# michaelriedl/2048-ppo-agent

Hardware: AMD Instinct MI355X
Metric: env-steps/sec at N parallel boards (full PPO loop: rollout with policy in the loop + GAE + update) (higher is better)
Workload: dtype u8 boards / bf16 policy; 1 GPU; 65536 parallel boards per GPU, Transformer policy bf16 (3.96 M params), full PPO iteration (BASELINE.json configs[2]; configs[3] when n_gpus=8); boards_per_gpu=65536, global_boards=65536, train_batch=2048, update_epochs=5, max_samples_per_epoch=300000, max_samples_per_epoch_is=global (each rank draws its 1/N share), as the reference's single subset, max_samples_per_epoch_per_rank=300000, rollout_mode=episodes (reference lock-step semantics), rng_mode=partitionable, parallelism=env-shard x1 + 1 grad all-reduce/minibatch

## Files before the change

2048-ppo-agent_amd/csrc/g2048_rowgemm.hip:

```cpp
#include <hip/hip_runtime.h>
#include <stdint.h>
#include <stdlib.h>

#include <type_traits>

#include "../../include/g2048.h"
#include "g2048_mfma.h"

namespace {

using namespace g2048_mfma;

constexpr int RG_N = 256, RG_KC = 128, RG_THREADS = 512, RG_WAVES = 8;
template <int NB> struct RgShape {
    static constexpr int TT = 32 * NB, STAGE = TT * RG_KC * 2, PIECES = TT * (RG_KC / 8) / RG_THREADS, RPW = TT / RG_WAVES, BATCH = RPW / 2;
    static constexpr int LDS = 2 * STAGE + RG_WAVES * 3 * RG_N * 4 + RG_N * 4;
    static_assert(PIECES * RG_THREADS == TT * (RG_KC / 8) && RPW % 2 == 0 && BATCH >= 1, "tile shape");
};

typedef uint32_t u32x4 __attribute__((ext_vector_type(4)));
enum { RG_FWD = 0, RG_BWD = 1 };

struct RowGemmArgs {
    const __bf16 *x;
// ... 312 lines not shown
                red[(w * 3 + 1) * RG_N + 4 * lane + q] = db[q];
                red[(w * 3 + 2) * RG_N + 4 * lane + q] = dsum[q];
            }
            lds_barrier();
            for (int c = tid; c < 3 * RG_N; c += RG_THREADS) {
                float s = 0.f;
#pragma unroll
                for (int ww = 0; ww < RG_WAVES; ++ww) s += red[ww * 3 * RG_N + c];
                float *dst = A.partial + (int64_t)blockIdx.x * 3 * RG_N + c;
                *dst = (tile == (int64_t)blockIdx.x) ? s : *dst + s;
            }
        }
    }
}

inline int rg_done() {
    const hipError_t e = hipGetLastError();
    return e == hipSuccess ? 0 : -(1000 + (int)e);
}

inline int rg_tpw(int64_t T, int *nb) {
    const char *e = getenv("G2048_RG_TWO_TILES");
    const bool two = e && e[0] == '1';
    int64_t t = (T + 255) / 256;
    if (two) t = (T + 511) / 512;
    if (t <= 96 && (two || t <= 48)) {
        *nb = 3;
        return (int)(t < 32 ? 32 : t);
    }
    *nb = 5;
// ... 45 lines not shown
extern "C" int g2048_linear_add_ln_fwd(const void *u, int64_t ldu, const void *w_packed, const float *bias, int K, const float *x,
                                       int64_t x_row_stride, const float *gamma, const float *beta, float *x_new, void *h, float *mean,
                                       float *rstd, int64_t T, float eps, float p_drop, uint64_t seed, const uint64_t *seed_state,
                                       void *stream) {
    if (!rg_gemm_ok(u, ldu, w_packed, T, K) || !x || !gamma || !beta || !x_new || !h || !mean || !rstd || !(p_drop >= 0.f && p_drop < 1.f) ||
        (x_row_stride & 3) || (((uintptr_t)x | (uintptr_t)gamma | (uintptr_t)beta | (uintptr_t)x_new | (uintptr_t)bias) & 15) ||
        ((uintptr_t)h & 7))
        return G2048_EINVAL;
    RowGemmArgs A{};
    A.x = (const __bf16 *)u; A.ldx = ldu; A.w = (const __bf16 *)w_packed; A.bias = bias; A.T = T; A.K = K;
    A.w_tile_stride = (int64_t)(K >> 4) * 512; A.extra_period = 1;
    A.res = x; A.res_rs = x_row_stride; A.gamma = gamma; A.beta = beta; A.mean = mean; A.rstd = rstd; A.out_f32 = x_new;
    A.out_bf16 = (uint16_t *)h; A.eps = eps; A.inv_keep = 1.0f / (1.0f - p_drop); A.thr = (uint32_t)(p_drop * 16777216.0f);
    A.s0 = (uint32_t)seed; A.s1 = (uint32_t)(seed >> 32); A.seed_state = seed_state; A.g_x_period = 1;
    return rg_launch<RG_FWD>(A, (hipStream_t)stream);
}

extern "C" int g2048_linear_add_ln_bwd(const void *dy, int64_t lddy, const void *wt_packed, int64_t wt_tile_stride, int K,
                                       const float *x_norm, int64_t x_row_stride, const float *g_x, int g_x_period, const void *g_h_extra,
                                       int extra_period, const float *mean, const float *rstd, const float *gamma, float *dx, void *da,
                                       float *partial, int64_t T, float p_drop, uint64_t seed, const uint64_t *seed_state, void *stream) {
    if (wt_tile_stride == 0) wt_tile_stride = (int64_t)(K >> 4) * 512;
    if (wt_tile_stride < (int64_t)(K >> 4) * 512 || (wt_tile_stride & 7) || (g_h_extra && extra_period < 1) || ((uintptr_t)g_h_extra & 7))
        return G2048_EINVAL;
    if (!rg_gemm_ok(dy, lddy, wt_packed, T, K) || !x_norm || !mean || !rstd || !gamma || !dx || !partial || g_x_period < 1 ||
        !(p_drop >= 0.f && p_drop < 1.f) || (x_row_stride & 3) ||
        (((uintptr_t)x_norm | (uintptr_t)g_x | (uintptr_t)gamma | (uintptr_t)dx) & 15) || ((uintptr_t)da & 7) || ((uintptr_t)partial & 3))
        return G2048_EINVAL;
    RowGemmArgs A{};
    A.x = (const __bf16 *)dy; A.ldx = lddy; A.w = (const __bf16 *)wt_packed; A.T = T; A.K = K;
// ... 8 lines not shown
```

2048-ppo-agent_amd/src/g2048/native.py:

```python
from __future__ import annotations

import ctypes as C
import os

import numpy as np
import torch

RNG_LEGACY = 0
RNG_PARTITIONABLE = 1
POLICY_DRUL = 0
POLICY_RANDOM = 1
MAX_FUSED_STEPS = 128

_PKG_ROOT = os.path.abspath(os.path.join(os.path.dirname(__file__), "..", ".."))
LIB_PATH = os.environ.get("G2048_LIB", os.path.join(_PKG_ROOT, "lib", "libg2048.so"))

_u32, _i32, _i64, _vp, _dbl = C.c_uint32, C.c_int, C.c_int64, C.c_void_p, C.c_double

SIGNATURES = {
    "g2048_abi_version": [],
    "g2048_split": [_u32, _u32, _vp, _i64, _i32, _vp],
    "g2048_chain_keys": [_vp, _vp, _i64, _i32],
    "g2048_init": [_vp, _vp, _vp, _vp, _i64, _i32, _vp],
    "g2048_step": [_vp, _vp, _vp, _vp, _vp, _vp, _i64, _i32, _vp],
# ... 28 lines not shown
    "g2048_linear_relu_dropout_bf16": [_vp, _i64, _vp, _i64, _vp, _vp, _i64, _i64, _i32, _i32, C.c_float, C.c_uint64, _vp, _vp, _vp],
    "g2048_linear_mask_bwd_workspace_floats": [_i64, _i32],
    "g2048_linear_mask_bwd_bf16": [_vp, _i64, _vp, _i64, _vp, _vp, _i64, _vp, _vp, _i64, _i32, _i32, C.c_float, _vp],
    "g2048_embed_fwd": [_vp, _vp, C.c_int, _vp, _vp, _vp, _i64, C.c_float, C.c_uint64, _vp, _vp],
    "g2048_embed_ln_fwd": [_vp, _vp, C.c_int, _vp, _vp, _vp, _i64, C.c_float, C.c_uint64, _vp, _vp, _vp, C.c_float, _vp, _vp, _vp, _vp],
    "g2048_embed_bwd_workspace_floats": [_i64],
    "g2048_embed_bwd": [_vp, _vp, _vp, _vp, _i64, C.c_float, C.c_uint64, _vp, _vp],
    "g2048_gather_minibatch": [_vp, _i64, _i64] + [_vp] * 13,
    "g2048_colsum_workspace_floats": [_i64, _i32],
    "g2048_colsum": [_vp, _i32, _i64, _i64, _i32, _vp, _vp, _vp],
    "g2048_colsum_partial_rows": [_i64, _i32],
    "g2048_linear_mask_bwd_partial_rows": [_i64, _i32],
    "g2048_reduce_jobs": [_vp, _i32, _vp],
    "g2048_linear_add_ln_fwd": [_vp, _i64, _vp, _vp, _i32, _vp, _i64, _vp, _vp, _vp, _vp, _vp, _vp, _i64, C.c_float, C.c_float,
                                C.c_uint64, _vp, _vp],
    "g2048_linear_add_ln_bwd_partial_rows": [_i64],
    "g2048_linear_add_ln_bwd": [_vp, _i64, _vp, _i64, _i32, _vp, _i64, _vp, _i32, _vp, _i32, _vp, _vp, _vp, _vp, _vp, _vp, _i64,
                                C.c_float, C.c_uint64, _vp, _vp],
    "g2048_mlp_embed_fwd": [_vp, _vp, _vp, _vp, _vp, _i64, _vp],
    "g2048_gemm_jobs": [_vp, _i32, _i64, _vp],
    "g2048_mlp_out_fwd": [_vp, _vp, _vp, _vp, _i64, _vp],
    "g2048_mlp_out_bwd_partial_rows": [_i64],
    "g2048_mlp_out_bwd": [_vp, _vp, _vp, _vp, _vp, _vp, _i64, _vp],
    "g2048_add_ln_bwd_workspace_floats": [_i64],
    "g2048_add_ln_bwd": [_vp, _i64, _vp, _vp, _vp, _vp, _vp, _vp, _vp, _vp, _vp, _i64, C.c_float, C.c_uint64, _vp,
                         _i32, _vp],
    "g2048_relu_dropout_fwd": [_vp, _vp, _i64, _i32, C.c_float, C.c_uint64, _vp, _vp],
    "g2048_relu_dropout_bwd_workspace_floats": [_i64, _i32],
    "g2048_relu_dropout_bwd": [_vp, _vp, _vp, _vp, _vp, _i64, _i32, C.c_float, _vp],
    "g2048_cls_tail_fwd": [_vp, _vp, _i64, _vp, _vp, _vp, _vp, _i64, C.c_float, C.c_float, C.c_uint64, _vp, _vp],
# ... 288 lines not shown


def rowgemm_ok(u2: torch.Tensor, w_packed: torch.Tensor, tile_stride: int = 0) -> bool:
    if u2.dim() != 2 or not u2.is_cuda or u2.dtype != torch.bfloat16 or u2.stride(1) != 1:
        return False
    T, K = u2.shape
    span = 256 * K if not tile_stride else 7 * int(tile_stride) + (K // 16) * 512
    return (T > 0 and K % 256 == 0 and 256 <= K <= 1024 and u2.stride(0) >= K and u2.stride(0) % 8 == 0 and u2.data_ptr() % 16 == 0
            and w_packed is not None and w_packed.is_cuda and w_packed.dtype == torch.bfloat16 and w_packed.is_contiguous()
            and (w_packed.numel() == span if not tile_stride else (w_packed.numel() >= span and tile_stride >= (K // 16) * 512
                                                                  and tile_stride % 8 == 0))
            and w_packed.data_ptr() % 16 == 0 and 160 * u2.stride(0) * 2 < 2 ** 31)


def linear_add_ln_fwd(u2, w_packed, bias, x_ptr: int, x_row_stride: int, gamma, beta, x_new, h, mean, rstd, eps: float,
                      p_drop: float, seed: int, seed_state: int = 0):
    if not rowgemm_ok(u2, w_packed):
        raise NativeError(f"linear_add_ln_fwd: operands {tuple(u2.shape)} (strides {u2.stride()}) x packed {w_packed.numel()} not supported")
    T, K = u2.shape
    bf = torch.bfloat16
    _check(load().g2048_linear_add_ln_fwd(u2.data_ptr(), u2.stride(0), w_packed.data_ptr(), _dev(bias, f32, 256, "bias", optional=True),
                                          K, x_ptr, int(x_row_stride), _dev(gamma, f32, 256, "gamma"), _dev(beta, f32, 256, "beta"),
                                          _dev(x_new, f32, 256 * T, "x_new"), _dev(h, bf, 256 * T, "h"), _dev(mean, f32, T, "mean"),
                                          _dev(rstd, f32, T, "rstd"), T, float(eps), float(p_drop), int(seed), seed_state or None,
                                          _stream()), "g2048_linear_add_ln_fwd")


def linear_add_ln_bwd(dy2, wt_packed, xn_ptr: int, x_row_stride: int, g_x, mean, rstd, gamma, dx, da, p_drop: float, seed: int,
                      seed_state: int = 0, g_x_period: int = 1, tile_stride: int = 0, g_h_extra=None, extra_period: int = 1):
    if not rowgemm_ok(dy2, wt_packed, tile_stride):
        raise NativeError(f"linear_add_ln_bwd: operands {tuple(dy2.shape)} (strides {dy2.stride()}) x packed {wt_packed.numel()} not supported")
# ... 157 lines not shown
    if logits.numel() != 4 * M or values.numel() != M:
        raise NativeError(f"ppo_loss: logits {tuple(logits.shape)} / values {tuple(values.shape)} do not match M={M}")
    new_logp = torch.empty(M, dtype=f32, device=logits.device)
    sums = torch.empty(5, dtype=f32, device=logits.device)
    dlogits, dvalues = torch.empty_like(logits), torch.empty_like(values)
    _check(load().g2048_ppo_loss(
        logits.data_ptr(), int(logits.dtype == torch.bfloat16), values.data_ptr(), int(values.dtype == torch.bfloat16),
        _dev(actions, u8, M, "actions"), _dev(mask_bits, u8, M, "mask_bits", optional=True), _dev(old_logp, f32, M, "old_logp"),
        _dev(adv, f32, M, "adv"), _dev(ret, f32, M, "ret"), M, float(clip_eps), float(c_value), float(c_entropy),
        new_logp.data_ptr(), sums.data_ptr(), dlogits.data_ptr(), dvalues.data_ptr(),
        _dev(grad_scale, f32, 1, "grad_scale", optional=True), _dev(running, torch.float64, 5, "running", optional=True),
        _stream()), "g2048_ppo_loss")
    return new_logp, sums, dlogits, dvalues


def linear_ok(x2: torch.Tensor, weight: torch.Tensor) -> bool:
    return (x2.is_cuda and x2.dtype == torch.bfloat16 and weight.dtype == torch.bfloat16 and x2.dim() == 2
            and weight.dim() == 2 and x2.stride(1) == 1 and weight.stride(1) == 1 and x2.shape[1] == weight.shape[1]
            and x2.shape[1] % 128 == 0 and weight.shape[0] % 128 == 0 and x2.stride(0) % 8 == 0 and weight.stride(0) % 8 == 0
            and x2.data_ptr() % 16 == 0 and weight.data_ptr() % 16 == 0 and x2.shape[0] > 0)


def linear_bf16(x2: torch.Tensor, weight: torch.Tensor, bias_f32=None, out=None) -> torch.Tensor:
    if not linear_ok(x2, weight):
        raise NativeError(f"linear_bf16: unsupported operands {tuple(x2.shape)} {x2.dtype} x {tuple(weight.shape)} {weight.dtype}")
    T, K = x2.shape
    N = weight.shape[0]
    if out is None:
        out = torch.empty((T, N), dtype=torch.bfloat16, device=x2.device)
    _check(load().g2048_linear_bf16(x2.data_ptr(), x2.stride(0), weight.data_ptr(), weight.stride(0),
# ... 317 lines not shown
```

2048-ppo-agent_amd/src/ppo/hip_ops.py:

```python
import weakref

import torch
import torch.nn as nn
import torch.nn.functional as F


class Bf16Shadow:

    _live = weakref.WeakSet()

    def __init__(self, params, transposed=(), packed=(), packed_only=(), packed_t_only=()):
        self.params = list(params)
        self.key, self.flat, self.views = None, None, None
        self.transposed = tuple(transposed)
        self.tviews = {}
        self.packed = tuple(packed)
        self.packed_only, self.packed_t_only = tuple(packed_only), tuple(packed_t_only)
        self.pviews, self.ptviews = {}, {}
        self.maintainer = None
        Bf16Shadow._live.add(self)

    def __getstate__(self):
        return {"params": self.params, "transposed": self.transposed, "packed": self.packed, "packed_only": self.packed_only,
                "packed_t_only": self.packed_t_only}
# ... 200 lines not shown

    def take(self):
        p, self.pending = self.pending, None
        return p


class FFNLink:

    __slots__ = ("p_drop", "db", "masked", "bias_param", "db_sunk", "bits")

    def __init__(self, p_drop: float):
        self.p_drop, self.db, self.masked = float(p_drop), None, False
        self.bits = None
        self.bias_param, self.db_sunk = None, False



_SINK_SLICES = 16


def _dweight_parts(dy2: torch.Tensor, x2: torch.Tensor) -> torch.Tensor:
    T, S = x2.shape[0], _SINK_SLICES
    if T >= 16384:
        from ..g2048 import native as nv

        slices = 16 if dy2.shape[1] * x2.shape[1] > 256 * 256 else 32
        if nv.dweight_ok(dy2, x2, slices):
            return nv.dweight_parts(dy2, x2, slices, block_rows=128)
    if T % S == 0 and T // S >= 64:
        return torch.bmm(dy2.view(S, T // S, -1).transpose(1, 2), x2.view(S, T // S, -1))
# ... 400 lines not shown

    @staticmethod
    def backward(ctx, g):
        if ctx.link is not None:
            ctx.link.g = g.contiguous()
            return None, None
        gx = g.new_zeros(ctx.shape)
        gx[:, :1] = g
        return gx, None


class _LinearAddLayerNorm(torch.autograd.Function):

    @staticmethod
    def forward(ctx, u, weight, bias, wb, bb, x, gamma, beta, eps, p_drop, wbT=None, link=None, cls_link=None, h_link=None,
                w_packed=None):
        from ..g2048 import native as nv

        ctx.set_materialize_grads(False)
        ctx.wbT, ctx.link = wbT, link
        ctx.params = (weight, bias, gamma, beta)
        ctx.cls_link = cls_link
        ctx.h_link = h_link
        if h_link is not None:
            h_link.armed = _rowgemm_on()
        if cls_link is not None:
            cls_link.attached = x.dim() == 3
        x, row_stride = _residual_rows(x)
        T = x.numel() // 256
        gamma, beta = gamma.contiguous(), beta.contiguous()
        h = torch.empty(x.shape, dtype=torch.bfloat16, device=x.device)
        x_new = torch.empty(x.shape, dtype=torch.float32, device=x.device)
        stats = torch.empty((2, T), dtype=torch.float32, device=x.device)
        seed = _seed_pair(x, p_drop)
        u2 = u.reshape(-1, u.shape[-1])
        if (w_packed is not None and _rowgemm_on() and u2.shape[0] == T and T >= 4096 and (bias is None or bias.dtype == torch.float32)
                and nv.rowgemm_ok(u2, w_packed)):
            nv.linear_add_ln_fwd(u2, w_packed, None if bias is None else bias.detach(), x.data_ptr(), row_stride, gamma, beta, x_new, h,
                                 stats[0], stats[1], eps, p_drop, *seed)
        else:
            with torch.autocast("cuda", enabled=False):
                a = _hip_linear(u2, wb, bias.detach()) if bias is not None and u.is_contiguous() else None
                a = F.linear(u, wb, bb) if a is None else a.view(*u.shape[:-1], wb.shape[0])
            nv.add_ln_fwd(x.data_ptr(), row_stride, a, gamma, beta, x_new, h, stats[0], stats[1], T, eps, p_drop, *seed)
        ctx.save_for_backward(u, wb, x_new, gamma, stats)
        ctx.meta = (p_drop, seed)
        return x_new, h

    @staticmethod
    def backward(ctx, g_x, g_h):
        from ..g2048 import native as nv
# ... 37 lines not shown
                if link is not None and link.bits is not None and ctx.wbT is not None and _stationary_ok(da2, ctx.wbT):
                    sink1 = _sink_for(link.bias_param)
                    if sink1 is not None:
                        du, ws1 = nv.linear_mask_bwd(da2, ctx.wbT, link.bits, link.p_drop, final=False)
                        sink1.add(link.bias_param, ws1, ws1.shape[1], ws1.shape[1], ws1.shape[0])
                        link.db, link.db_sunk = None, True
                    else:
                        du, link.db = nv.linear_mask_bwd(da2, ctx.wbT, link.bits, link.p_drop)
                    link.masked, link.bits = True, None
                    du = du.view(u.shape)
                else:
                    du = _hip_linear(da2, ctx.wbT) if ctx.wbT is not None else None
                    du = (da2 @ wb if du is None else du).view(u.shape)
            if sink is not None:
                _sink_weight(sink, weight, da2, u2)
                return du, None, None, None, None, dx, None, None, None, None, None, None, None, None, None
            dw = _dweight(da2, u2)
        return du, dw, dparams[2], None, None, dx, dparams[0], dparams[1], None, None, None, None, None, None, None


class _LinearAddCast(torch.autograd.Function):

    @staticmethod
    def forward(ctx, u, weight, bias, wb, bb, x, p_drop):
        from ..g2048 import native as nv

        with torch.autocast("cuda", enabled=False):
            a = F.linear(u, wb, bb)
        ctx.params = (weight, bias)
        xr, row_stride = _residual_rows(x)
        T = xr.numel() // 256
        h = torch.empty(xr.shape, dtype=torch.bfloat16, device=x.device)
        seed = _seed_pair(xr, p_drop)
# ... 17 lines not shown
        ws = nv.add_ln_bwd(0, 256, None, g_h.contiguous(), None, None, None, dx, da, dparams, T, p_drop, *seed)
        with torch.autocast("cuda", enabled=False):
            da2, u2 = da.view(T, 256), u.reshape(T, -1)
            du = (da2 @ wb).view(u.shape) if ctx.needs_input_grad[0] else None
            if sink is not None:
                sink.add(bias, ws[:, 512:], 768, 256, ws.shape[0])
                _sink_weight(sink, weight, da2, u2)
                return du, None, None, None, None, dx, None
            dw = _dweight(da2, u2)
        return du, dw, dparams[2], None, None, dx, None


class _LinearReluDropout(torch.autograd.Function):

    @staticmethod
    def forward(ctx, h, weight, bias, wb, bb, p_drop, link=None, h_link=None, wt_packed=None):
        from ..g2048 import native as nv

        ctx.h_link, ctx.wt_packed = h_link, wt_packed
        h2 = h.reshape(-1, h.shape[-1])
        with torch.autocast("cuda", enabled=False):
            if _stationary_ok(h2, wb) and bias.dtype == torch.float32:
                y = nv.linear_relu_dropout(h2, wb, bias.detach(), p_drop, *_seed_pair(h2, p_drop), want_mask=link is not None)
                if link is not None:
                    y, link.bits = y
                y = y.view(*h.shape[:-1], wb.shape[0])
            else:
                z = _hip_linear(h2, wb, bias)
                z = F.linear(h, wb, bb) if z is None else z.view(*h.shape[:-1], wb.shape[0])
                y = torch.empty_like(z)
                nv.relu_dropout_fwd(z, y, p_drop, *_seed_pair(z, p_drop))
        ctx.save_for_backward(h, wb, y)
        ctx.p_drop, ctx.link = p_drop, link
        ctx.params = (weight, bias)
        if link is not None:
            link.bias_param = bias
        return y
# ... 14 lines not shown
            dz = torch.empty_like(y)
            db = None if sink is not None else torch.empty(y.shape[-1], dtype=torch.float32, device=y.device)
            ws = nv.relu_dropout_bwd(dy.contiguous(), y, dz, db, ctx.p_drop)
            if sink is not None:
                sink.add(bias, ws, ws.shape[1], ws.shape[1], ws.shape[0])
                db_done = True
        with torch.autocast("cuda", enabled=False):
            dz2, h2 = dz.view(-1, dz.shape[-1]), h.reshape(-1, h.shape[-1])
            dh = None
            if ctx.needs_input_grad[0] and not (ctx.h_link is not None and ctx.h_link.offer(dz2, ctx.wt_packed)):
                dh = (dz2 @ wb).view(h.shape)
            if sink is not None:
                _sink_weight(sink, weight, dz2, h2)
                if not db_done:
                    sink.add(bias, db.contiguous(), db.numel(), db.numel(), 1)
                return dh, None, None, None, None, None, None, None, None
            dw = _dweight(dz2, h2)
        return dh, dw, (None if db_done else db), None, None, None, None, None, None


def _fused_norm_ok(x: torch.Tensor, a) -> bool:
    return (x.is_cuda and x.dtype == torch.float32 and x.shape[-1] == 256 and torch.is_grad_enabled()
            and torch.is_autocast_enabled() and torch.get_autocast_dtype("cuda") == torch.bfloat16
            and (a is None or a.dtype == torch.bfloat16))


def _add_norm(x: torch.Tensor, a, norm: nn.LayerNorm, p: float, training: bool, h_link=None, pre=None):
    if _fused_norm_ok(x, a):
        if a is None and _residual_rows(x)[0] is not x:
            return x, _AddLayerNorm.apply(x, a, norm.weight, norm.bias, norm.eps, 0.0)[1]
        return _AddLayerNorm.apply(x, a, norm.weight, norm.bias, norm.eps, p if training else 0.0, h_link, pre)
    if a is not None:
        x = x + F.dropout(a, p, training)
# ... 199 lines not shown
```

2048-ppo-agent_amd/src/ppo/transformer_encoder.py:

```python
import math
import os

import torch
import torch.nn as nn
import torch.nn.functional as F

from ..env_definitions import BOARD_DIM
from .hip_ops import (Bf16Shadow, ClsLink, FFNLink, HLink, LNPre, _AddLayerNorm, _ClsRows, _AttnCls, _AttnPacked, _EmbedBoards, _ExpandRows, _InProjCls,
                      _LinearAddCast, _LinearAddLayerNorm, _LinearReluDropout, _LinearSplitK, _add_norm, _fused_attention_ok, _fused_norm_ok,
                      _linear, _train_bf16, graph_seed_state)



def get_emb(sin_inp: torch.Tensor) -> torch.Tensor:
    return torch.stack((sin_inp.sin(), sin_inp.cos()), dim=-1).flatten(-2, -1)


class PositionalEncoding2D(nn.Module):

    def __init__(self, x_size, y_size, channels, dropout=0.1, dtype_override=None):
        super().__init__()
        self.org_channels = channels
        self.dtype_override = dtype_override
        self.channels = int(math.ceil(channels / 4) * 2)
# ... 25 lines not shown
    def __init__(self, d_model: int, nhead: int, num_layers: int, dim_feedforward: int, dropout: float = 0.1):
        super().__init__()
        self.d_model, self.nhead, self.num_layers = d_model, nhead, num_layers
        self.dim_feedforward, self.dropout = dim_feedforward, dropout
        self.positional_encoding = PositionalEncoding2D(BOARD_DIM[0], BOARD_DIM[1], channels=d_model, dropout=dropout)
        self.cls_token = nn.Parameter(torch.randn(1, 1, d_model))
        self._shadow = None
        self.encoder = nn.TransformerEncoder(
            nn.TransformerEncoderLayer(d_model=d_model, nhead=nhead, dim_feedforward=dim_feedforward, dropout=dropout,
                                       norm_first=True, batch_first=True),
            num_layers=num_layers, enable_nested_tensor=False)

    def _bf16_weights(self, like: torch.Tensor):
        layers = self.encoder.layers
        if not _train_bf16(like, layers[0].linear1.weight):
            return [[None] * 14 for _ in layers]
        if self._shadow is None:
            ps = []
            for l in layers:
                ps += [l.self_attn.in_proj_weight, l.self_attn.in_proj_bias, l.self_attn.out_proj.weight,
                       l.self_attn.out_proj.bias, l.linear1.weight, l.linear1.bias, l.linear2.weight, l.linear2.bias]
            last = len(layers) - 1
            fuse = range(last) if self.d_model == 256 else range(0)
            self._shadow = Bf16Shadow(ps, transposed=[8 * i + 6 for i in range(len(layers))] + [8 * i + 2 for i in range(last)],
                                      packed=[8 * last + 2, 8 * last + 4, 8 * last + 6],
                                      packed_only=[8 * i + o for i in fuse for o in (2, 6)],
                                      packed_t_only=[8 * i + o for i in fuse for o in (0, 4)] + ([8 * last] if self.d_model == 256 and last >= 1 else []))
        v = self._shadow()
        tv, pv, ptv = self._shadow.tviews, self._shadow.pviews, self._shadow.ptviews
        full = range(len(layers) - 1)
        return [v[8 * i:8 * i + 8] + [tv[8 * i + 6], tv.get(8 * i + 2)]
                + ([pv.get(8 * i + 2), pv.get(8 * i + 6), ptv.get(8 * i + 0), ptv.get(8 * i + 4)] if i in full
                   else [None, None, ptv.get(8 * i + 0), None])
                for i in range(len(layers))]

    def _layer(self, layer: nn.TransformerEncoderLayer, x: torch.Tensor, h: torch.Tensor, next_norm,
               cls_only: bool = False, sh=(None,) * 14, cls_link_out=None, cls_link_in=None, tail_heads=None, h_link_in=None,
               h_link_out=None):
        B, S, D = x.shape
        H = self.nhead
        p = self.dropout if self.training else 0.0
        attn = layer.self_attn
        if cls_only:
            w, b = attn.in_proj_weight, attn.in_proj_bias
            if sh[0] is not None and h.dtype == torch.bfloat16:
                q, kv = _InProjCls.apply(h, w, b, sh[0], sh[1], h_link_in, sh[12])
            else:
                q = _linear(h[:, :1], w[:D], b[:D])
                kv = _linear(h, w[D:], b[D:])
            x = _ClsRows.apply(x, cls_link_in) if cls_link_in is not None else x[:, :1]
            if _fused_attention_ok(kv, S, D // H):
                a = _AttnCls.apply(q, kv, H, p)
# ... 14 lines not shown
            i_last = len(self.encoder.layers) - 1
            pv, ptv = self._shadow.pviews, self._shadow.ptviews
            n2 = layer.norm2
            return tail_heads(a, x, dict(wo=attn.out_proj.weight, bo=attn.out_proj.bias, ln_g=n2.weight, ln_b=n2.bias,
                                         w1=layer.linear1.weight, b1=layer.linear1.bias, w2=layer.linear2.weight,
                                         b2=layer.linear2.bias),
                              {k: pv[8 * i_last + o] for k, o in (("wo", 2), ("w1", 4), ("w2", 6))},
                              {k: ptv[8 * i_last + o] for k, o in (("wo", 2), ("w1", 4), ("w2", 6))}, n2.eps, p), None
        if sh[0] is not None and a.dtype == torch.bfloat16 and _fused_norm_ok(x, None) \
                and layer.linear1.out_features % 8 == 0 and layer.linear1.out_features <= 2048:
            n2 = layer.norm2
            mid = HLink() if sh[13] is not None else None
            x, h = _LinearAddLayerNorm.apply(a, attn.out_proj.weight, attn.out_proj.bias, sh[2], sh[3], x, n2.weight,
                                             n2.bias, n2.eps, p, sh[9], None, None, mid, sh[10])
            link = FFNLink(p) if next_norm is not None else None
            f = _LinearReluDropout.apply(h, layer.linear1.weight, layer.linear1.bias, sh[4], sh[5], p, link, mid, sh[13])
            if next_norm is None:
                if sh[6] is not None and layer.linear2.bias is not None:
                    return _LinearAddCast.apply(f, layer.linear2.weight, layer.linear2.bias, sh[6], sh[7], x, p), None
                f = _linear(f, layer.linear2.weight, layer.linear2.bias, sh[6], sh[7])
                return x + F.dropout(f, p, self.training), None
            return _LinearAddLayerNorm.apply(f, layer.linear2.weight, layer.linear2.bias, sh[6], sh[7], x, next_norm.weight,
                                             next_norm.bias, next_norm.eps, p, sh[8], link, cls_link_out, h_link_out, sh[11])
        a = _linear(a, attn.out_proj.weight, attn.out_proj.bias, sh[2], sh[3])
        x, h = _add_norm(x, a, layer.norm2, p, self.training)
        f = F.dropout(F.relu(_linear(h, layer.linear1.weight, layer.linear1.bias, sh[4], sh[5])), p, self.training)
        f = _linear(f, layer.linear2.weight, layer.linear2.bias, sh[6], sh[7])
        if next_norm is None:
            return x + F.dropout(f, p, self.training), None
        return _add_norm(x, f, next_norm, p, self.training)

    def forward(self, src: torch.Tensor, reduction: str = "mean") -> torch.Tensor:
        if reduction not in ["mean", "cls"]:
            raise ValueError(f"reduction must be 'mean' or 'cls', got {reduction}")
        x = self.positional_encoding.forward_flat(src)
        x = torch.cat([_ExpandRows.apply(self.cls_token.to(x.dtype), x.shape[0]), x], dim=1)
        return self.encode(x, reduction)

# ... 34 lines not shown
```

include/g2048.h:

```cpp
#ifndef G2048_H
#define G2048_H

#include <stdint.h>

#ifdef __cplusplus
extern "C" {
#endif

#define G2048_ABI_VERSION 4
#define G2048_EINVAL (-1)
#define G2048_RNG_LEGACY 0
#define G2048_RNG_PARTITIONABLE 1
#define G2048_POLICY_DRUL 0
#define G2048_POLICY_RANDOM 1
#define G2048_MAX_FUSED_STEPS 128

int g2048_abi_version(void);


int g2048_split(uint32_t key0, uint32_t key1, uint32_t *out_keys, int64_t n, int rng_mode, void *stream);

int g2048_chain_keys(uint32_t *key , uint32_t *subs , int64_t n, int rng_mode);


// ... 72 lines not shown
                   void *stream);


int g2048_add_ln_fwd(const float *x, int64_t x_row_stride, const void *a, const float *gamma, const float *beta,
                     float *x_new, void *h, float *mean, float *rstd, int64_t T, float eps, float p_drop,
                     uint64_t seed, const uint64_t *seed_state, void *stream);
int64_t g2048_add_ln_bwd_workspace_floats(int64_t T);
int g2048_add_ln_bwd(const float *x_norm, int64_t x_row_stride, const float *g_x, const void *g_h, const float *mean,
                     const float *rstd, const float *gamma, float *dx, void *da, float *dparams, float *workspace,
                     int64_t T, float p_drop, uint64_t seed, const uint64_t *seed_state, int g_x_period, void *stream);


int g2048_linear_add_ln_fwd(const void *u, int64_t ldu, const void *w_packed, const float *bias, int K, const float *x,
                            int64_t x_row_stride, const float *gamma, const float *beta, float *x_new, void *h, float *mean,
                            float *rstd, int64_t T, float eps, float p_drop, uint64_t seed, const uint64_t *seed_state, void *stream);
int64_t g2048_linear_add_ln_bwd_partial_rows(int64_t T);
int g2048_linear_add_ln_bwd(const void *dy, int64_t lddy, const void *wt_packed, int64_t wt_tile_stride, int K, const float *x_norm,
                            int64_t x_row_stride, const float *g_x, int g_x_period, const void *g_h_extra, int extra_period,
                            const float *mean, const float *rstd, const float *gamma, float *dx, void *da, float *partial, int64_t T,
                            float p_drop, uint64_t seed, const uint64_t *seed_state, void *stream);


int g2048_mlp_embed_fwd(const uint8_t *boards, const void *wt, const float *bias, void *y, void *onehot, int64_t M, void *stream);

#define G2048_GEMM_MAX_JOBS 8
typedef struct {
    const void *x[2]; int64_t ldx[2];
    const void *w[2]; int64_t ldw[2];
    int32_t k[2];
    const float *bias;
// ... 144 lines not shown
```

Before: 3.749 million env-steps/sec.

## Fuse FFN linear1+ReLU+dropout with linear2+residual+LayerNorm in one chained kernel

Adds a persistent HIP kernel that computes the first FFN GEMM with ReLU and dropout per 160-token tile in LDS, chunk by chunk, and feeds each chunk straight into the second GEMM. The residual add and LayerNorm epilogue run in the same kernel. The Python autograd path defers linear1 via an FFNChain object so linear2+LN can launch the fused kernel. The intermediate activation z and the mask bits are still written for backward. This removes a kernel launch and the re-read of the 1024-wide intermediate from global memory, at the cost of heavy register and LDS pressure and a complex double-buffered schedule.

```diff
diff --git a/2048-ppo-agent_amd/csrc/g2048_rowgemm.hip b/2048-ppo-agent_amd/csrc/g2048_rowgemm.hip
--- a/2048-ppo-agent_amd/csrc/g2048_rowgemm.hip
+++ b/2048-ppo-agent_amd/csrc/g2048_rowgemm.hip
@@ -350,6 +350,264 @@
     }
 }
 
+constexpr int FC_U1 = 160 * 512, FC_STAGE = 160 * 256, FC_LDS = FC_U1 + 2 * FC_STAGE;
+
+__device__ __forceinline__ uint32_t fc_opaque(uint32_t v) {
+    asm volatile("" : "+v"(v));
+    return v;
+}
+
+struct FfnChainArgs {
+    RowGemmArgs rg;
+    const __bf16 *u1;
+    int64_t ldu1;
+    const __bf16 *w1;
+    const float *b1;
+    uint16_t *z;
+    uint32_t *bits;
+    float inv_keep1;
+    uint32_t thr16, s0, s1;
+    const uint64_t *seed_state1;
+};
+
+template <int NCH>
+__global__ void __launch_bounds__(RG_THREADS, 2)
+k_ffn_chain(FfnChainArgs F) {
+    constexpr int NB = 5, TT = RgShape<NB>::TT, RPW = RgShape<NB>::RPW, BATCH = RgShape<NB>::BATCH;
+    const RowGemmArgs &A = F.rg;
+    extern __shared__ __attribute__((aligned(16))) char smem[];
+    char *const u1s = smem;
+    const int tid = threadIdx.x, lane = tid & 63, r = lane & 31, h = lane >> 5;
+    const int w = __builtin_amdgcn_readfirstlane(tid >> 6);
+    uint32_t s0 = A.s0, s1 = A.s1;
+    if (A.seed_state) {
+        const uint64_t s = *A.seed_state;
+        s0 ^= (uint32_t)s * 0x9E3779B1u;
+        s1 += (uint32_t)(s >> 32) * 0x85EBCA77u + (uint32_t)s;
+    }
+    uint32_t e0 = F.s0, e1 = F.s1;
+    if (F.seed_state1) {
+        const uint64_t sd = *F.seed_state1;
+        e0 ^= (uint32_t)sd * 0x9E3779B1u;
+        e1 += (uint32_t)(sd >> 32) * 0x85EBCA77u + (uint32_t)sd;
+    }
+    const uint32_t hi_term = e0 ^ (e1 * 0x85EBCA77u);
+    const int64_t n_tiles = (A.T + A.tpw - 1) / A.tpw;
+    const int64_t t_pad = (A.T + 63) & ~(int64_t)63;
+    const int f = w & 3;
+    const uint32_t lane16 = (uint32_t)lane * 16;
+    const uint32_t zoff = (uint32_t)((tid >> 4) * 2048 + 16 * (tid & 15));
+    const uint32_t urow = (uint32_t)(r * 512), ux = (uint32_t)(((h ^ r) & 15) << 4);
+    const uint32_t srow = (uint32_t)(r * 256 + 8 * h), sx = (uint32_t)(((4 * f) ^ (r & 15)) << 4);
+
+    for (int64_t tile = blockIdx.x; tile < n_tiles; tile += gridDim.x) {
+        const int64_t tok0 = tile * A.tpw;
+        const int n_valid = (int)((A.T - tok0 < A.tpw) ? A.T - tok0 : A.tpw);
+        {
+            const int row0 = tid >> 5, pc = tid & 31;
+            const uint32_t lo = (uint32_t)(row0 * 512 + (((pc & 16) | ((pc ^ row0) & 15)) << 4));
+            u32x4 v[10];
+#pragma unroll
+            for (int j = 0; j < 10; ++j) {
+                const int row = row0 + 16 * j;
+                v[j] = *reinterpret_cast<const u32x4 *>(F.u1 + (tok0 + (row < n_valid ? row : n_valid - 1)) * F.ldu1 + 8 * pc);
+            }
+            lds_barrier();
+#pragma unroll
+            for (int j = 0; j < 10; ++j) *reinterpret_cast<u32x4 *>(u1s + lo + j * 16 * 512) = v[j];
+        }
+        constexpr int W1R = 16;
+        bf16x8 W1r[W1R];
+        auto w1_frag = [&](unsigned cc, int ks) __attribute__((always_inline)) {
+            return *reinterpret_cast<const bf16x8 *>(reinterpret_cast<const char *>(F.w1) + ((size_t)(4 * cc + f) * 16 + ks) * 1024 + lane16);
+        };
+        f32x16 bias1;
+        auto w1_head = [&](unsigned cc) __attribute__((always_inline)) {
+#pragma unroll
+            for (int ks = 0; ks < W1R; ++ks) W1r[ks] = w1_frag(cc, ks);
+            bias1 = bias_tile(F.b1, 128 * (int)cc + 32 * f, h);
+        };
+        auto lin1_blocks = [&](unsigned cc, char *st, auto b0_c, auto nbk_c) __attribute__((always_inline)) {
+            constexpr int B0 = decltype(b0_c)::value, NBK = decltype(nbk_c)::value;
+            const int nw = 128 * (int)cc + 32 * f;
+            const uint32_t ur = fc_opaque(urow), uxx = fc_opaque(ux);
+            auto frag = [&](int j, int ks) __attribute__((always_inline)) {
+                return *reinterpret_cast<const bf16x8 *>(u1s + 16384 * (B0 + j) + 256 * (ks >> 3) + ur + ((32u * (ks & 7)) ^ uxx));
+            };
+            const uint32_t sr = fc_opaque(srow), sxx = fc_opaque(sx);
+#pragma unroll
+            for (int j = 0; j < NBK; ++j) {
+                f32x16 acc = bias1;
+                constexpr int PRE = 3;
+                bf16x8 q[PRE];
+#pragma unroll
+                for (int ks = 0; ks < PRE; ++ks) q[ks] = frag(j, ks);
+#pragma unroll
+                for (int ks = 0; ks < 16; ++ks) {
+                    __builtin_amdgcn_sched_barrier(0);
+                    acc = mfma(W1r[ks], q[ks % PRE], acc);
+                    if (ks + PRE < 16) q[ks % PRE] = frag(j, ks + PRE);
+                }
+                __builtin_amdgcn_sched_barrier(0);
+                const int b = B0 + j, row = 32 * b + r;
+                const bool valid = row < n_valid;
+                const int64_t tok = tok0 + (valid ? row : n_valid - 1);
+                const uint32_t pair0 = (uint32_t)(((uint64_t)tok * 1024u + (uint64_t)(nw + 4 * h)) >> 1);
+#pragma unroll
+                for (int pi = 0; pi < 8; ++pi) {
+                    const int i = 2 * pi;
+                    uint32_t xh = (pair0 + (uint32_t)(((i & 3) >> 1) + 4 * (i >> 2))) * 0x9E3779B1u + hi_term;
+                    xh ^= xh >> 16; xh *= 0x7FEB352Du; xh ^= xh >> 15; xh *= 0x846CA68Bu; xh ^= xh >> 16;
+                    const uint32_t keep = ((xh & 0xFFFFu) >= F.thr16 ? 1u : 0u) | ((xh >> 16) >= F.thr16 ? 2u : 0u);
+                    const float a = fmaxf(acc[i], 0.f), c = fmaxf(acc[i + 1], 0.f);
+                    acc[i] = (keep & 1u) ? a * F.inv_keep1 : 0.f;
+                    acc[i + 1] = (keep & 2u) ? c * F.inv_keep1 : 0.f;
+                }
+                uint32_t obits = 0u;
+#pragma unroll
+                for (int g = 0; g < 4; ++g) {
+                    const uint32_t lo = f2bf(acc[4 * g + 0]) | (f2bf(acc[4 * g + 1]) << 16);
+                    const uint32_t hi = f2bf(acc[4 * g + 2]) | (f2bf(acc[4 * g + 3]) << 16);
+                    obits |= (((lo & 0x7FFFu) ? 1u : 0u) | ((lo & 0x7FFF0000u) ? 2u : 0u) | ((hi & 0x7FFFu) ? 4u : 0u) |
+                              ((hi & 0x7FFF0000u) ? 8u : 0u)) << (4 * g);
+                    *reinterpret_cast<uint2 *>(st + 8192 * b + sr + ((16u * g) ^ sxx)) = make_uint2(lo, hi);
+                }
+                if (F.bits && valid) {
+                    auto put = [&](int64_t t) __attribute__((always_inline)) {
+                        const uint32_t word = (uint32_t)(((t >> 6) * 4) * 512 + 32 * h + (t & 31)), half = (uint32_t)((t >> 5) & 1);
+                        *reinterpret_cast<uint16_t *>(reinterpret_cast<char *>(F.bits) + ((size_t)(cc >> 1) * 512 + 64 * (4 * (cc & 1) + f)) * 4 +
+                                                      (4 * word + 2 * half)) = (uint16_t)obits;
+                    };
+                    put(tok);
+                    if (tok == A.T - 1)
+                        for (int64_t t = A.T; t < t_pad; ++t) put(t);
+                }
+            }
+        };
+        auto lin1 = [&](unsigned cc, char *st) __attribute__((always_inline)) {
+            if (w < 4) lin1_blocks(cc, st, std::integral_constant<int, 0>{}, std::integral_constant<int, 3>{});
+            else lin1_blocks(cc, st, std::integral_constant<int, 3>{}, std::integral_constant<int, 2>{});
+        };
+        constexpr int WR = 4, NG = 8 * NCH;
+        const char *const wp = reinterpret_cast<const char *>(A.w + (size_t)w * A.w_tile_stride);
+        bf16x8 W[WR];
+        const uint32_t brow0 = (uint32_t)(r * (RG_KC * 2)), bx0 = (uint32_t)((h ^ (r & 15)) << 4);
+        unsigned kc = 0;
+        w1_head(0);
+#pragma unroll
+        for (int g = 0; g < WR; ++g) W[g] = *reinterpret_cast<const bf16x8 *>(wp + (size_t)g * 1024 + lane16);
+        f32x16 acc[NB];
+        lds_barrier();
+        lin1(0, smem + FC_U1);
+        lds_barrier();
+#pragma unroll
+        for (int b = 0; b < NB; ++b) acc[b] = A.bias ? bias_tile(A.bias, 32 * w, h) : zero_tile();
+#define FC_FRAG(st, s_) \
+    *reinterpret_cast<const bf16x8 *>((st) + brow + ((32u * ((s_) / NB)) ^ bx) + ((s_) % NB) * (32 * RG_KC * 2))
+#define FC_CHUNK(c)                                                                                                        \
+    if constexpr ((c) < NCH) {                                                                                             \
+        char *const st = smem + FC_U1 + ((c) & 1) * FC_STAGE;                                                              \
+        const uint32_t brow = fc_opaque(brow0), bx = fc_opaque(bx0), zo = fc_opaque(zoff);                                 \
+        if constexpr ((c) + 1 < NCH) w1_head(kc + 1);                                                                      \
+        constexpr int PRE = 3, NS = 8 * NB;                                                                                \
+        bf16x8 q[PRE];                                                                                                     \
+        _Pragma("unroll") for (int s_ = 0; s_ < PRE; ++s_) q[s_] = FC_FRAG(st, s_);                                        \
+        _Pragma("unroll") for (int s_ = 0; s_ < NS; ++s_) {                                                                \
+            __builtin_amdgcn_sched_barrier(0);                                                                             \
+            const int ks = s_ / NB, b = s_ % NB, g = 8 * (c) + ks;                                                         \
+            acc[b] = mfma(W[g % WR], q[s_ % PRE], acc[b]);                                                                 \
+            if (s_ + PRE < NS) q[s_ % PRE] = FC_FRAG(st, s_ + PRE);                                                        \
+            if (b == NB - 1 && g + WR < NG) W[g % WR] = *reinterpret_cast<const bf16x8 *>(wp + (size_t)(kc * 8 + ks + WR) * 1024 + lane16); \
+        }                                                                                                                  \
+        __builtin_amdgcn_sched_barrier(0);                                                                                 \
+        {         \
+            const int row0 = tid >> 4, p = tid & 15;                                                                       \
+            u32x4 v[5];                                                                                                    \
+            _Pragma("unroll") for (int i = 0; i < 5; ++i)                                                                  \
+                v[i] = *reinterpret_cast<const u32x4 *>(st + (row0 + 32 * i) * 256 + ((p ^ (row0 & 15)) << 4));          \
+            _Pragma("unroll") for (int i = 0; i < 5; ++i)                                                                  \
+                if (row0 + 32 * i < n_valid)                                                                               \
+                    *reinterpret_cast<u32x4 *>(reinterpret_cast<char *>(F.z) + ((tok0 + 32 * i) * 1024 + 128 * (c)) * 2 + zo) = v[i]; \
+        }                                                                                                                  \
+        if constexpr ((c) + 1 < NCH) lin1(kc + 1, smem + FC_U1 + (((c) + 1) & 1) * FC_STAGE);                             \
+        kc += 1;                                                                                                           \
+        asm volatile("" : "+s"(kc));                                                                                       \
+        lds_barrier();                                                                                                     \
+    }
+        FC_CHUNK(0) FC_CHUNK(1) FC_CHUNK(2) FC_CHUNK(3) FC_CHUNK(4) FC_CHUNK(5) FC_CHUNK(6) FC_CHUNK(7)
+#undef FC_CHUNK
+#undef FC_FRAG
+
+#pragma unroll
+        for (int b = 0; b < NB; ++b) {
+            const int trow = 32 * b + r;
+#pragma unroll
+            for (int g = 0; g < 4; ++g) {
+                const uint32_t lo = f2bf(acc[b][4 * g + 0]) | (f2bf(acc[b][4 * g + 1]) << 16);
+                const uint32_t hi = f2bf(acc[b][4 * g + 2]) | (f2bf(acc[b][4 * g + 3]) << 16);
+                *reinterpret_cast<uint2 *>(smem + trow * 512 + (((4 * w + g) ^ (trow & 31)) << 4) + 8 * h) = make_uint2(lo, hi);
+            }
+        }
+        lds_barrier();
+        const float4 gm = reinterpret_cast<const float4 *>(A.gamma)[lane];
+        const float4 bt = reinterpret_cast<const float4 *>(A.beta)[lane];
+        float4 fv[RPW];
+#pragma unroll
+        for (int j = 0; j < RPW; ++j) {
+            const int row = w + RG_WAVES * j;
+            fv[j] = reinterpret_cast<const float4 *>(A.res + (tok0 + (row < n_valid ? row : n_valid - 1)) * A.res_rs)[lane];
+        }
+#pragma unroll
+        for (int j0 = 0; j0 < RPW; j0 += BATCH) {
+            if (w + RG_WAVES * j0 >= n_valid) break;
+            float4 v[BATCH];
+            float s[BATCH];
+#pragma unroll
+            for (int j = 0; j < BATCH; ++j) {
+                const int row = w + RG_WAVES * (j0 + j), rowc = row < n_valid ? row : n_valid - 1;
+                const int64_t tok = tok0 + rowc;
+                const uint2 ab = *reinterpret_cast<const uint2 *>(smem + rowc * 512 + ((((lane >> 1) ^ (rowc & 31))) << 4) + 8 * (lane & 1));
+                float av[4] = {bf2f(ab.x & 0xFFFFu), bf2f(ab.x >> 16), bf2f(ab.y & 0xFFFFu), bf2f(ab.y >> 16)};
+                if (A.thr) {
+                    const uint64_t base = (uint64_t)tok * RG_N + 4 * lane;
+#pragma unroll
+                    for (int q = 0; q < 4; ++q) av[q] = keep_elem(s0, s1, A.thr, base + q) ? av[q] * A.inv_keep : 0.0f;
+                }
+                v[j] = fv[j0 + j];
+                v[j].x += av[0]; v[j].y += av[1]; v[j].z += av[2]; v[j].w += av[3];
+                if (row < n_valid) reinterpret_cast<float4 *>(A.out_f32 + tok * RG_N)[lane] = v[j];
+                s[j] = v[j].x + v[j].y + v[j].z + v[j].w;
+            }
+#pragma unroll
+            for (int j = 0; j < BATCH; ++j) s[j] = wave_sum_dpp(s[j]);
+            float mean[BATCH];
+#pragma unroll
+            for (int j = 0; j < BATCH; ++j) {
+                mean[j] = s[j] * (1.0f / RG_N);
+                v[j].x -= mean[j]; v[j].y -= mean[j]; v[j].z -= mean[j]; v[j].w -= mean[j];
+                s[j] = v[j].x * v[j].x + v[j].y * v[j].y + v[j].z * v[j].z + v[j].w * v[j].w;
+            }
+#pragma unroll
+            for (int j = 0; j < BATCH; ++j) s[j] = wave_sum_dpp(s[j]);
+#pragma unroll
+            for (int j = 0; j < BATCH; ++j) {
+                const int row = w + RG_WAVES * (j0 + j);
+                const int64_t tok = tok0 + row;
+                const float rstd = rsqrtf(s[j] * (1.0f / RG_N) + A.eps);
+                const uint32_t lo = f2bf(v[j].x * rstd * gm.x + bt.x) | (f2bf(v[j].y * rstd * gm.y + bt.y) << 16);
+                const uint32_t hi = f2bf(v[j].z * rstd * gm.z + bt.z) | (f2bf(v[j].w * rstd * gm.w + bt.w) << 16);
+                if (row < n_valid) {
+                    reinterpret_cast<uint2 *>(A.out_bf16 + tok * RG_N)[lane] = make_uint2(lo, hi);
+                    if (lane == 0) {
+                        A.mean[tok] = mean[j];
+                        A.rstd[tok] = rstd;
+                    }
+                }
+            }
+        }
+    }
+}
+
 inline int rg_done() {
     const hipError_t e = hipGetLastError();
     return e == hipSuccess ? 0 : -(1000 + (int)e);
@@ -425,6 +683,37 @@
     A.out_bf16 = (uint16_t *)h; A.eps = eps; A.inv_keep = 1.0f / (1.0f - p_drop); A.thr = (uint32_t)(p_drop * 16777216.0f);
     A.s0 = (uint32_t)seed; A.s1 = (uint32_t)(seed >> 32); A.seed_state = seed_state; A.g_x_period = 1;
     return rg_launch<RG_FWD>(A, (hipStream_t)stream);
+}
+
+extern "C" int g2048_ffn_chain_fwd(const void *u1, int64_t ldu1, const void *w1_packed, const float *b1, void *z, void *mask_bits,
+                                   uint64_t seed1, const uint64_t *seed_state1, const void *w2_packed, const float *b2, const float *x,
+                                   int64_t x_row_stride, const float *gamma, const float *beta, float *x_new, void *h, float *mean,
+                                   float *rstd, int64_t T, float eps, float p_drop, uint64_t seed2, const uint64_t *seed_state2,
+                                   void *stream) {
+    if (!u1 || !w1_packed || !b1 || !z || !w2_packed || !x || !gamma || !beta || !x_new || !h || !mean || !rstd || T <= 0 ||
+        !(p_drop >= 0.f && p_drop < 1.f) || ldu1 < 256 || (ldu1 & 7) || (x_row_stride & 3) || 160 * ldu1 * 2 >= (1ll << 31) ||
+        (((uintptr_t)u1 | (uintptr_t)w1_packed | (uintptr_t)b1 | (uintptr_t)z | (uintptr_t)w2_packed | (uintptr_t)b2 | (uintptr_t)x |
+          (uintptr_t)gamma | (uintptr_t)beta | (uintptr_t)x_new) & 15) ||
+        (((uintptr_t)h | (uintptr_t)mask_bits) & 7))
+        return G2048_EINVAL;
+    FfnChainArgs F{};
+    RowGemmArgs &A = F.rg;
+    A.ldx = 1024; A.w = (const __bf16 *)w2_packed; A.bias = b2; A.T = T; A.K = 1024;
+    A.w_tile_stride = (int64_t)(1024 >> 4) * 512; A.extra_period = 1;
+    A.res = x; A.res_rs = x_row_stride; A.gamma = gamma; A.beta = beta; A.mean = mean; A.rstd = rstd; A.out_f32 = x_new;
+    A.out_bf16 = (uint16_t *)h; A.eps = eps; A.inv_keep = 1.0f / (1.0f - p_drop); A.thr = (uint32_t)(p_drop * 16777216.0f);
+    A.s0 = (uint32_t)seed2; A.s1 = (uint32_t)(seed2 >> 32); A.seed_state = seed_state2; A.g_x_period = 1;
+    F.u1 = (const __bf16 *)u1; F.ldu1 = ldu1; F.w1 = (const __bf16 *)w1_packed; F.b1 = b1; F.z = (uint16_t *)z;
+    F.bits = (uint32_t *)mask_bits; F.inv_keep1 = 1.0f / (1.0f - p_drop); F.thr16 = (uint32_t)(p_drop * 65536.0f + 0.5f);
+    F.s0 = (uint32_t)seed1; F.s1 = (uint32_t)(seed1 >> 32); F.seed_state1 = p_drop > 0.f ? seed_state1 : nullptr;
+    int64_t t = (T + 255) / 256;
+    A.tpw = (int)(t < 32 ? 32 : t > 160 ? 160 : t);
+    const int64_t tiles = (T + A.tpw - 1) / A.tpw;
+    const unsigned grid = (unsigned)(tiles < 256 ? tiles : 256);
+    const void *fn = reinterpret_cast<const void *>(k_ffn_chain<8>);
+    if (hipFuncSetAttribute(fn, hipFuncAttributeMaxDynamicSharedMemorySize, FC_LDS) != hipSuccess) return -(1000 + (int)hipGetLastError());
+    hipLaunchKernelGGL((k_ffn_chain<8>), dim3(grid), dim3(RG_THREADS), FC_LDS, (hipStream_t)stream, F);
+    return rg_done();
 }
 
 extern "C" int g2048_linear_add_ln_bwd(const void *dy, int64_t lddy, const void *wt_packed, int64_t wt_tile_stride, int K,
diff --git a/2048-ppo-agent_amd/src/g2048/native.py b/2048-ppo-agent_amd/src/g2048/native.py
--- a/2048-ppo-agent_amd/src/g2048/native.py
+++ b/2048-ppo-agent_amd/src/g2048/native.py
@@ -66,6 +66,8 @@
     "g2048_reduce_jobs": [_vp, _i32, _vp],
     "g2048_linear_add_ln_fwd": [_vp, _i64, _vp, _vp, _i32, _vp, _i64, _vp, _vp, _vp, _vp, _vp, _vp, _i64, C.c_float, C.c_float,
                                 C.c_uint64, _vp, _vp],
+    "g2048_ffn_chain_fwd": [_vp, _i64, _vp, _vp, _vp, _vp, C.c_uint64, _vp, _vp, _vp, _vp, _i64, _vp, _vp, _vp, _vp, _vp, _vp, _i64,
+                            C.c_float, C.c_float, C.c_uint64, _vp, _vp],
     "g2048_linear_add_ln_bwd_partial_rows": [_i64],
     "g2048_linear_add_ln_bwd": [_vp, _i64, _vp, _i64, _i32, _vp, _i64, _vp, _i32, _vp, _i32, _vp, _vp, _vp, _vp, _vp, _vp, _i64,
                                 C.c_float, C.c_uint64, _vp, _vp],
@@ -384,7 +386,11 @@
 
 
 def linear_add_ln_fwd(u2, w_packed, bias, x_ptr: int, x_row_stride: int, gamma, beta, x_new, h, mean, rstd, eps: float,
-                      p_drop: float, seed: int, seed_state: int = 0):
+                      p_drop: float, seed: int, seed_state: int = 0, lin1=None):
+    if lin1 is not None:
+        u1, w1_packed, b1, mask, seed1, seed_state1 = lin1
+        return ffn_chain_fwd(u1, w1_packed, b1, u2, mask, seed1, seed_state1, w_packed, bias, x_ptr, x_row_stride, gamma, beta, x_new,
+                             h, mean, rstd, eps, p_drop, seed, seed_state)
     if not rowgemm_ok(u2, w_packed):
         raise NativeError(f"linear_add_ln_fwd: operands {tuple(u2.shape)} (strides {u2.stride()}) x packed {w_packed.numel()} not supported")
     T, K = u2.shape
@@ -572,6 +578,31 @@
     return new_logp, sums, dlogits, dvalues
 
 
+def ffn_chain_ok(u1: torch.Tensor, w1_packed, w2_packed) -> bool:
+    return (u1.dim() == 2 and u1.is_cuda and u1.dtype == torch.bfloat16 and u1.shape[1] == 256 and u1.stride(1) == 1
+            and u1.shape[0] > 0 and u1.stride(0) >= 256 and u1.stride(0) % 8 == 0 and u1.data_ptr() % 16 == 0
+            and 160 * u1.stride(0) * 2 < 2 ** 31
+            and all(w is not None and w.is_cuda and w.dtype == torch.bfloat16 and w.is_contiguous() and w.numel() == 1024 * 256
+                    and w.data_ptr() % 16 == 0 for w in (w1_packed, w2_packed)))
+
+
+def ffn_chain_fwd(u1, w1_packed, b1, z, mask, seed1: int, seed_state1: int, w2_packed, b2, x_ptr: int, x_row_stride: int, gamma, beta,
+                  x_new, h, mean, rstd, eps: float, p_drop: float, seed2: int, seed_state2: int = 0):
+    if not ffn_chain_ok(u1, w1_packed, w2_packed):
+        raise NativeError(f"ffn_chain_fwd: operands {tuple(u1.shape)} (strides {u1.stride()}) not supported")
+    T = u1.shape[0]
+    bf = torch.bfloat16
+    if mask is not None and (mask.dtype != u8 or not mask.is_cuda or mask.numel() != load().g2048_ffn_mask_bytes(T, 1024)):
+        raise NativeError(f"ffn_chain_fwd: the mask does not belong to a [{T}, 1024] forward call")
+    _check(load().g2048_ffn_chain_fwd(u1.data_ptr(), u1.stride(0), w1_packed.data_ptr(), _dev(b1, f32, 1024, "b1"),
+                                      _dev(z, bf, 1024 * T, "z"), None if mask is None else mask.data_ptr(), int(seed1) & (2 ** 64 - 1),
+                                      seed_state1 or None, w2_packed.data_ptr(), _dev(b2, f32, 256, "b2", optional=True), x_ptr,
+                                      int(x_row_stride), _dev(gamma, f32, 256, "gamma"), _dev(beta, f32, 256, "beta"),
+                                      _dev(x_new, f32, 256 * T, "x_new"), _dev(h, bf, 256 * T, "h"), _dev(mean, f32, T, "mean"),
+                                      _dev(rstd, f32, T, "rstd"), T, float(eps), float(p_drop), int(seed2) & (2 ** 64 - 1),
+                                      seed_state2 or None, _stream()), "g2048_ffn_chain_fwd")
+
+
 def linear_ok(x2: torch.Tensor, weight: torch.Tensor) -> bool:
     return (x2.is_cuda and x2.dtype == torch.bfloat16 and weight.dtype == torch.bfloat16 and x2.dim() == 2
             and weight.dim() == 2 and x2.stride(1) == 1 and weight.stride(1) == 1 and x2.shape[1] == weight.shape[1]
diff --git a/2048-ppo-agent_amd/src/ppo/hip_ops.py b/2048-ppo-agent_amd/src/ppo/hip_ops.py
--- a/2048-ppo-agent_amd/src/ppo/hip_ops.py
+++ b/2048-ppo-agent_amd/src/ppo/hip_ops.py
@@ -238,6 +238,30 @@
         self.bits = None
         self.bias_param, self.db_sunk = None, False
 
+
+
+def _ffn_chain_on() -> bool:
+    import os
+
+    return os.environ.get("G2048_FFN_CHAIN", "0").strip().lower() in ("1", "true", "yes", "on")
+
+
+class FFNChain:
+
+    __slots__ = ("w1_packed", "pending")
+
+    def __init__(self, w1_packed):
+        self.w1_packed, self.pending = w1_packed, None
+
+    def usable(self, h2: torch.Tensor, wb: torch.Tensor, bias) -> bool:
+        from ..g2048 import native as nv
+
+        return (_ffn_chain_on() and _rowgemm_on() and tuple(wb.shape) == (1024, 256) and h2.shape[0] >= 4096 and bias is not None
+                and bias.dtype == torch.float32 and _stationary_ok(h2, wb) and nv.ffn_chain_ok(h2, self.w1_packed, self.w1_packed))
+
+    def take(self):
+        p, self.pending = self.pending, None
+        return p
 
 
 _SINK_SLICES = 16
@@ -668,7 +692,7 @@
 
     @staticmethod
     def forward(ctx, u, weight, bias, wb, bb, x, gamma, beta, eps, p_drop, wbT=None, link=None, cls_link=None, h_link=None,
-                w_packed=None):
+                w_packed=None, chain=None):
         from ..g2048 import native as nv
 
         ctx.set_materialize_grads(False)
@@ -688,7 +712,14 @@
         stats = torch.empty((2, T), dtype=torch.float32, device=x.device)
         seed = _seed_pair(x, p_drop)
         u2 = u.reshape(-1, u.shape[-1])
-        if (w_packed is not None and _rowgemm_on() and u2.shape[0] == T and T >= 4096 and (bias is None or bias.dtype == torch.float32)
+        pend = chain.take() if chain is not None else None
+        if pend is not None:
+            h1, b1, bits, seed1 = pend
+            if not (u2.shape[0] == T and bias is not None and bias.dtype == torch.float32 and nv.ffn_chain_ok(h1, chain.w1_packed, w_packed)):
+                raise RuntimeError("FFNChain: the linked linear2 cannot take the chained launch")
+            nv.linear_add_ln_fwd(u2, w_packed, bias.detach(), x.data_ptr(), row_stride, gamma, beta, x_new, h, stats[0], stats[1], eps,
+                                 p_drop, *seed, lin1=(h1, chain.w1_packed, b1, bits, *seed1))
+        elif (w_packed is not None and _rowgemm_on() and u2.shape[0] == T and T >= 4096 and (bias is None or bias.dtype == torch.float32)
                 and nv.rowgemm_ok(u2, w_packed)):
             nv.linear_add_ln_fwd(u2, w_packed, None if bias is None else bias.detach(), x.data_ptr(), row_stride, gamma, beta, x_new, h,
                                  stats[0], stats[1], eps, p_drop, *seed)
@@ -756,9 +787,9 @@
                     du = (da2 @ wb if du is None else du).view(u.shape)
             if sink is not None:
                 _sink_weight(sink, weight, da2, u2)
-                return du, None, None, None, None, dx, None, None, None, None, None, None, None, None, None
+                return du, None, None, None, None, dx, None, None, None, None, None, None, None, None, None, None
             dw = _dweight(da2, u2)
-        return du, dw, dparams[2], None, None, dx, dparams[0], dparams[1], None, None, None, None, None, None, None
+        return du, dw, dparams[2], None, None, dx, dparams[0], dparams[1], None, None, None, None, None, None, None, None
 
 
 class _LinearAddCast(torch.autograd.Function):
@@ -806,13 +837,19 @@
 class _LinearReluDropout(torch.autograd.Function):
 
     @staticmethod
-    def forward(ctx, h, weight, bias, wb, bb, p_drop, link=None, h_link=None, wt_packed=None):
+    def forward(ctx, h, weight, bias, wb, bb, p_drop, link=None, h_link=None, wt_packed=None, chain=None):
         from ..g2048 import native as nv
 
         ctx.h_link, ctx.wt_packed = h_link, wt_packed
         h2 = h.reshape(-1, h.shape[-1])
         with torch.autocast("cuda", enabled=False):
-            if _stationary_ok(h2, wb) and bias.dtype == torch.float32:
+            if link is not None and chain is not None and chain.usable(h2, wb, bias):
+                T = h2.shape[0]
+                y = torch.empty((T, 1024), dtype=torch.bfloat16, device=h.device)
+                link.bits = torch.empty(nv.load().g2048_ffn_mask_bytes(T, 1024), dtype=torch.uint8, device=h.device)
+                chain.pending = (h2, bias.detach(), link.bits, _seed_pair(h2, p_drop))
+                y = y.view(*h.shape[:-1], 1024)
+            elif _stationary_ok(h2, wb) and bias.dtype == torch.float32:
                 y = nv.linear_relu_dropout(h2, wb, bias.detach(), p_drop, *_seed_pair(h2, p_drop), want_mask=link is not None)
                 if link is not None:
                     y, link.bits = y
@@ -857,9 +894,9 @@
                 _sink_weight(sink, weight, dz2, h2)
                 if not db_done:
                     sink.add(bias, db.contiguous(), db.numel(), db.numel(), 1)
-                return dh, None, None, None, None, None, None, None, None
+                return dh, None, None, None, None, None, None, None, None, None
             dw = _dweight(dz2, h2)
-        return dh, dw, (None if db_done else db), None, None, None, None, None, None
+        return dh, dw, (None if db_done else db), None, None, None, None, None, None, None
 
 
 def _fused_norm_ok(x: torch.Tensor, a) -> bool:
diff --git a/2048-ppo-agent_amd/src/ppo/transformer_encoder.py b/2048-ppo-agent_amd/src/ppo/transformer_encoder.py
--- a/2048-ppo-agent_amd/src/ppo/transformer_encoder.py
+++ b/2048-ppo-agent_amd/src/ppo/transformer_encoder.py
@@ -6,7 +6,7 @@
 import torch.nn.functional as F
 
 from ..env_definitions import BOARD_DIM
-from .hip_ops import (Bf16Shadow, ClsLink, FFNLink, HLink, LNPre, _AddLayerNorm, _ClsRows, _AttnCls, _AttnPacked, _EmbedBoards, _ExpandRows, _InProjCls,
+from .hip_ops import (Bf16Shadow, ClsLink, FFNChain, FFNLink, HLink, LNPre, _AddLayerNorm, _ClsRows, _AttnCls, _AttnPacked, _EmbedBoards, _ExpandRows, _InProjCls,
                       _LinearAddCast, _LinearAddLayerNorm, _LinearReluDropout, _LinearSplitK, _add_norm, _fused_attention_ok, _fused_norm_ok,
                       _linear, _train_bf16, graph_seed_state)
 
@@ -63,7 +63,7 @@
     def _bf16_weights(self, like: torch.Tensor):
         layers = self.encoder.layers
         if not _train_bf16(like, layers[0].linear1.weight):
-            return [[None] * 14 for _ in layers]
+            return [[None] * 15 for _ in layers]
         if self._shadow is None:
             ps = []
             for l in layers:
@@ -73,18 +73,18 @@
             fuse = range(last) if self.d_model == 256 else range(0)
             self._shadow = Bf16Shadow(ps, transposed=[8 * i + 6 for i in range(len(layers))] + [8 * i + 2 for i in range(last)],
                                       packed=[8 * last + 2, 8 * last + 4, 8 * last + 6],
-                                      packed_only=[8 * i + o for i in fuse for o in (2, 6)],
+                                      packed_only=[8 * i + o for i in fuse for o in (2, 4, 6)],
                                       packed_t_only=[8 * i + o for i in fuse for o in (0, 4)] + ([8 * last] if self.d_model == 256 and last >= 1 else []))
         v = self._shadow()
         tv, pv, ptv = self._shadow.tviews, self._shadow.pviews, self._shadow.ptviews
         full = range(len(layers) - 1)
         return [v[8 * i:8 * i + 8] + [tv[8 * i + 6], tv.get(8 * i + 2)]
-                + ([pv.get(8 * i + 2), pv.get(8 * i + 6), ptv.get(8 * i + 0), ptv.get(8 * i + 4)] if i in full
-                   else [None, None, ptv.get(8 * i + 0), None])
+                + ([pv.get(8 * i + 2), pv.get(8 * i + 6), ptv.get(8 * i + 0), ptv.get(8 * i + 4), pv.get(8 * i + 4)] if i in full
+                   else [None, None, ptv.get(8 * i + 0), None, None])
                 for i in range(len(layers))]
 
     def _layer(self, layer: nn.TransformerEncoderLayer, x: torch.Tensor, h: torch.Tensor, next_norm,
-               cls_only: bool = False, sh=(None,) * 14, cls_link_out=None, cls_link_in=None, tail_heads=None, h_link_in=None,
+               cls_only: bool = False, sh=(None,) * 15, cls_link_out=None, cls_link_in=None, tail_heads=None, h_link_in=None,
                h_link_out=None):
         B, S, D = x.shape
         H = self.nhead
@@ -129,14 +129,15 @@
             x, h = _LinearAddLayerNorm.apply(a, attn.out_proj.weight, attn.out_proj.bias, sh[2], sh[3], x, n2.weight,
                                              n2.bias, n2.eps, p, sh[9], None, None, mid, sh[10])
             link = FFNLink(p) if next_norm is not None else None
-            f = _LinearReluDropout.apply(h, layer.linear1.weight, layer.linear1.bias, sh[4], sh[5], p, link, mid, sh[13])
+            chain = FFNChain(sh[14]) if link is not None and sh[14] is not None and sh[11] is not None else None
+            f = _LinearReluDropout.apply(h, layer.linear1.weight, layer.linear1.bias, sh[4], sh[5], p, link, mid, sh[13], chain)
             if next_norm is None:
                 if sh[6] is not None and layer.linear2.bias is not None:
                     return _LinearAddCast.apply(f, layer.linear2.weight, layer.linear2.bias, sh[6], sh[7], x, p), None
                 f = _linear(f, layer.linear2.weight, layer.linear2.bias, sh[6], sh[7])
                 return x + F.dropout(f, p, self.training), None
             return _LinearAddLayerNorm.apply(f, layer.linear2.weight, layer.linear2.bias, sh[6], sh[7], x, next_norm.weight,
-                                             next_norm.bias, next_norm.eps, p, sh[8], link, cls_link_out, h_link_out, sh[11])
+                                             next_norm.bias, next_norm.eps, p, sh[8], link, cls_link_out, h_link_out, sh[11], chain)
         a = _linear(a, attn.out_proj.weight, attn.out_proj.bias, sh[2], sh[3])
         x, h = _add_norm(x, a, layer.norm2, p, self.training)
         f = F.dropout(F.relu(_linear(h, layer.linear1.weight, layer.linear1.bias, sh[4], sh[5])), p, self.training)
diff --git a/include/g2048.h b/include/g2048.h
--- a/include/g2048.h
+++ b/include/g2048.h
@@ -110,6 +110,10 @@
 int g2048_linear_add_ln_fwd(const void *u, int64_t ldu, const void *w_packed, const float *bias, int K, const float *x,
                             int64_t x_row_stride, const float *gamma, const float *beta, float *x_new, void *h, float *mean,
                             float *rstd, int64_t T, float eps, float p_drop, uint64_t seed, const uint64_t *seed_state, void *stream);
+int g2048_ffn_chain_fwd(const void *u1, int64_t ldu1, const void *w1_packed, const float *b1, void *z, void *mask_bits, uint64_t seed1,
+                        const uint64_t *seed_state1, const void *w2_packed, const float *b2, const float *x, int64_t x_row_stride,
+                        const float *gamma, const float *beta, float *x_new, void *h, float *mean, float *rstd, int64_t T, float eps,
+                        float p_drop, uint64_t seed2, const uint64_t *seed_state2, void *stream);
 int64_t g2048_linear_add_ln_bwd_partial_rows(int64_t T);
 int g2048_linear_add_ln_bwd(const void *dy, int64_t lddy, const void *wt_packed, int64_t wt_tile_stride, int K, const float *x_norm,
                             int64_t x_row_stride, const float *g_x, int g_x_period, const void *g_h_extra, int extra_period,
```

Result: no change. 3.754 million env-steps/sec, median of 3 (+0.2%).
